# AssafSinger94/dino-tracker

Hardware: AMD Instinct MI355X
Metric: query-points*frames/s (higher is better)
Workload: dtype mixed: fp16 ViT operands (one per value), f16 conv operands in Delta-DINO, f16 candidates + f32 deciders in the tracker; f32 accumulate; 1 GPU; 854x480x90 synthetic video (model res 854x476, 67x121 tokens, C=384), 1024 grid queries; 1 video(s) per step over 1 GPU(s); features=vit, mode=single, track_method=mfma, anchor_pairs=92091, correlation_maps_per_video=8380350, rccl_ranks=1, parallelism=video-parallel x1

## Files before the change

### dino_tracker_amd/csrc/vit.hip

```cpp
#include <stdlib.h>
#include "common.h"
#include "vit_attention4.h"
#include "vit_attention6.h"
#include "vit_gemm_common.h"
#include "vit_gemm_tiled.h"
#include "vit_gemm_ws.h"
#include "vit_gemm_wide.h"
#include "vit_split.h"

namespace {

__global__ __launch_bounds__(256) void patch_embed_kernel(const float* __restrict__ frames, const float* __restrict__ Wp,
                                                          const float* __restrict__ bp, const float* __restrict__ pos,
                                                          const float* __restrict__ cls_pos,
                                                          const float* __restrict__ mean_std, float* __restrict__ x,
                                                          int H, int W, int ph, int pw, int D, int patch, int stride,
                                                          int S) {
    const int HW = ph * pw;
    const int K = 3 * patch * patch;
    const int frame = blockIdx.z;
    const int tid = threadIdx.x, lane = tid & 63, w = tid >> 6;
    const int p0 = blockIdx.x * 64 + (w >> 1) * 32;
    const int n0 = blockIdx.y * 64 + (w & 1) * 32;
    const int li = lane & 31, lk = lane >> 5;
    const float* img = frames + (size_t)frame * 3 * H * W;
    const int p = min(p0 + li, HW - 1);
    const int pr = p / pw, pc = p % pw;
    const int n = min(n0 + li, D - 1);
    const float* wrow = Wp + (size_t)n * K;
    f16v acc;
#pragma unroll
    for (int r = 0; r < 16; ++r) acc[r] = 0.f;
    for (int k = lk; k < K; k += 2) {
        const int ch = k / (patch * patch), rem = k - ch * patch * patch;
        const int ky = rem / patch, kx = rem - ky * patch;
        const float px = img[((size_t)ch * H + pr * stride + ky) * W + pc * stride + kx];
        const float a = (px - mean_std[ch]) / mean_std[3 + ch];
        acc = __builtin_amdgcn_mfma_f32_32x32x2f32(a, wrow[k], acc, 0, 0, 0);
    }
    const int co = n0 + li;
    if (co < D) {
        const float b = bp[co];
#pragma unroll
        for (int r = 0; r < 16; ++r) {
            const int i = (r & 3) + 8 * (r >> 2) + 4 * lk;
            const int pp = p0 + i;
            if (pp < HW) x[((size_t)frame * S + 1 + pp) * D + co] = acc[r] + b + pos[(size_t)pp * D + co];
        }
    }
    if (blockIdx.x == 0 && (w >> 1) == 0 && lk == 0 && co < D) x[(size_t)frame * S * D + co] = cls_pos[co];
}

constexpr int PE_P = 14, PE_S = 7, PE_TOK = 128, PE_NF = 96;
constexpr int PE_ROWPX = (PE_TOK - 1) * PE_S + PE_P;
constexpr int PE_K = PE_P * PE_P * 4;
constexpr int PE_CK = 2 * PE_P * 4;
constexpr int PE_WP = PE_CK + 8;
constexpr float PE_WSCALE = 256.f;

__global__ __launch_bounds__(256) void frame_split4_kernel(const float* __restrict__ frames, const float* __restrict__ mean_std,
                                                           h4v* __restrict__ hi_, h4v* __restrict__ lo_, int H, int W,
                                                           long long npix) {
    const long long i = (long long)blockIdx.x * 256 + threadIdx.x;
    if (i >= npix) return;
    const long long f = i / ((long long)H * W), p = i - f * (long long)H * W;
    const float* fr = frames + f * 3 * (long long)H * W + p;
    h4v h, l;
#pragma unroll
    for (int c = 0; c < 3; ++c) {
        const float v = (fr[(long long)c * H * W] - mean_std[c]) / mean_std[3 + c];
        h[c] = (half_t)v;
        l[c] = (half_t)(v - (float)h[c]);
    }
    h[3] = (half_t)0.f;
    l[3] = (half_t)0.f;
    hi_[i] = h;
    lo_[i] = l;
}

__global__ void pack_patch_split_kernel(const float* __restrict__ w, int D, half_t* __restrict__ Wh, half_t* __restrict__ Wl) {
    const long long idx = (long long)blockIdx.x * 256 + threadIdx.x;
    if (idx >= (long long)D * PE_K) return;
    const int n = (int)(idx / PE_K), k = (int)(idx - (long long)n * PE_K);
    const int tap = k >> 2, c = k & 3;
    const float v = c < 3 ? w[((size_t)n * 3 + c) * (PE_P * PE_P) + tap] * PE_WSCALE : 0.f;
    const half_t h = (half_t)v;
    Wh[idx] = h;
    Wl[idx] = (half_t)(v - (float)h);
}

__global__ __launch_bounds__(256) void patch_embed_split_kernel(const h4v* __restrict__ in_hi, const h4v* __restrict__ in_lo,
                                                                const half_t* __restrict__ Wh, const half_t* __restrict__ Wl,
                                                                const float* __restrict__ bp, const float* __restrict__ pos,
                                                                const float* __restrict__ cls_pos, float* __restrict__ x,
                                                                int H, int W, int ph, int pw, int D, int S, int groups_x,
                                                                int units, int slabs) {
    __shared__ h4v Xh[2 * PE_ROWPX], Xl[2 * PE_ROWPX];
    __shared__ __attribute__((aligned(16))) half_t Wsh[PE_NF * PE_WP], Wsl[PE_NF * PE_WP];
    const int tid = threadIdx.x, lane = tid & 63, w = tid >> 6;
    const int per_xcd = (units + 7) / 8;
    const int within = blockIdx.x >> 3;
    const int unit = (blockIdx.x & 7) * per_xcd + within / slabs;
    if (within / slabs >= per_xcd || unit >= units) return;
    const int n0 = (within % slabs) * PE_NF;
    const int pc0 = (unit % groups_x) * PE_TOK, pr = (unit / groups_x) % ph;
    const size_t frame = unit / (groups_x * ph);
    const int li = lane & 31, hh = lane >> 5;
    const h4v* fh = in_hi + frame * (size_t)H * W;
    const h4v* fl = in_lo + frame * (size_t)H * W;
    const int tokl = w * 32 + li;
    f16v acc[3];
#pragma unroll
    for (int n = 0; n < 3; ++n)
#pragma unroll
        for (int r = 0; r < 16; ++r) acc[n][r] = 0.f;
    for (int c = 0; c < PE_P / 2; ++c) {
        __syncthreads();
        for (int idx = tid; idx < 2 * PE_ROWPX; idx += 256) {
            const int r = idx / PE_ROWPX, px = idx - r * PE_ROWPX;
            const size_t g = (size_t)(pr * PE_S + 2 * c + r) * W + min(pc0 * PE_S + px, W - 1);
            Xh[idx] = fh[g];
            Xl[idx] = fl[g];
        }
        for (int idx = tid; idx < PE_NF * (PE_CK / 8); idx += 256) {
            const int f = idx / (PE_CK / 8), piece = idx - f * (PE_CK / 8);
            const size_t src = (size_t)min(n0 + f, D - 1) * PE_K + c * PE_CK + piece * 8;
            *reinterpret_cast<uint4*>(Wsh + f * PE_WP + piece * 8) = *reinterpret_cast<const uint4*>(Wh + src);
            *reinterpret_cast<uint4*>(Wsl + f * PE_WP + piece * 8) = *reinterpret_cast<const uint4*>(Wl + src);
        }
        __syncthreads();
#pragma unroll
        for (int ls = 0; ls < PE_CK / 16; ++ls) {
            const int t0 = 2 * (2 * ls + hh);
            const int p0 = (t0 / PE_P) * PE_ROWPX + tokl * PE_S + t0 % PE_P;
            const h4v a0 = Xh[p0], a1 = Xh[p0 + 1], b0 = Xl[p0], b1 = Xl[p0 + 1];
            const h8 xh = {a0[0], a0[1], a0[2], a0[3], a1[0], a1[1], a1[2], a1[3]};
            const h8 xl = {b0[0], b0[1], b0[2], b0[3], b1[0], b1[1], b1[2], b1[3]};
#pragma unroll
            for (int n = 0; n < 3; ++n) {
                const int wo = (n * 32 + li) * PE_WP + ls * 16 + hh * 8;
                const h8 wh = *reinterpret_cast<const h8*>(Wsh + wo), wl = *reinterpret_cast<const h8*>(Wsl + wo);
                acc[n] = __builtin_amdgcn_mfma_f32_32x32x16_f16(xl, wh, acc[n], 0, 0, 0);
                acc[n] = __builtin_amdgcn_mfma_f32_32x32x16_f16(xh, wl, acc[n], 0, 0, 0);
                acc[n] = __builtin_amdgcn_mfma_f32_32x32x16_f16(xh, wh, acc[n], 0, 0, 0);
            }
        }
    }
#pragma unroll
    for (int n = 0; n < 3; ++n) {
        const int co = n0 + n * 32 + li;
        if (co >= D) continue;
        const float b = bp[co];
#pragma unroll
        for (int r = 0; r < 16; ++r) {
            const int pc = pc0 + w * 32 + (r & 3) + 8 * (r >> 2) + 4 * hh;
            if (pc < pw) {
                const int pp = pr * pw + pc;
                x[((size_t)frame * S + 1 + pp) * D + co] = acc[n][r] * (1.f / PE_WSCALE) + b + pos[(size_t)pp * D + co];
            }
        }
        if (pr == 0 && pc0 == 0 && w == 0 && hh == 0) x[(size_t)frame * S * D + co] = cls_pos[co];
    }
}

template <typename T>
__global__ __launch_bounds__(256) void layernorm_kernel(float* __restrict__ x, const T* __restrict__ delta,
                                                        const float* __restrict__ gam, const float* __restrict__ bet,
                                                        T* __restrict__ y, long long rows, int D, float eps,
                                                        int* __restrict__ overflow) {
    typedef typename Vec<T>::t8 T8;
    typedef typename Vec<T>::t4 T4;
    (void)sizeof(T8); (void)sizeof(T4);
    operand_mode<T>();
    const long long row = (long long)blockIdx.x * 4 + (threadIdx.x >> 6);
    if (row >= rows) return;
    const int lane = threadIdx.x & 63;
    float* p = x + row * D;
    float4 v[4];
    float s = 0.f;
    bool sat = false;
#pragma unroll
    for (int it = 0; it < 4; ++it) {
        const int c = lane * 4 + it * 256;
        if (c < D) {
            v[it] = *reinterpret_cast<const float4*>(p + c);
            if (delta) {
                const T4 d = *reinterpret_cast<const T4*>(delta + row * D + c);
                const float d0 = (float)d[0], d1 = (float)d[1], d2 = (float)d[2], d3 = (float)d[3];
                if (IsF16<T>::value) sat |= !(fmaxf(fmaxf(fabsf(d0), fabsf(d1)), fmaxf(fabsf(d2), fabsf(d3))) < 65504.f);
                v[it].x += d0; v[it].y += d1; v[it].z += d2; v[it].w += d3;
                *reinterpret_cast<float4*>(p + c) = v[it];
            }
            s += (v[it].x + v[it].y) + (v[it].z + v[it].w);
        }
    }
    if (IsF16<T>::value && overflow && __any(sat) && lane == 0) atomicOr(overflow, 1);
    const float mean = wave_sum(s) / (float)D;
    float q = 0.f;
#pragma unroll
    for (int it = 0; it < 4; ++it) {
        if (lane * 4 + it * 256 < D) {
            const float a = v[it].x - mean, b = v[it].y - mean, cc = v[it].z - mean, d = v[it].w - mean;
            q += (a * a + b * b) + (cc * cc + d * d);
        }
    }
    const float rstd = rsqrtf(wave_sum(q) / (float)D + eps);
    if (!y) return;
    T* o = y + row * D;
#pragma unroll
    for (int it = 0; it < 4; ++it) {
        const int c = lane * 4 + it * 256;
        if (c < D) {
            const float4 g = *reinterpret_cast<const float4*>(gam + c), b = *reinterpret_cast<const float4*>(bet + c);
            T4 r = {(T)((v[it].x - mean) * rstd * g.x + b.x), (T)((v[it].y - mean) * rstd * g.y + b.y),
                     (T)((v[it].z - mean) * rstd * g.z + b.z), (T)((v[it].w - mean) * rstd * g.w + b.w)};
            *reinterpret_cast<T4*>(o + c) = r;
        }
    }
}

__global__ __launch_bounds__(256) void zero_kernel(uint4* __restrict__ p, long long n16) {
    const long long i = (long long)blockIdx.x * 256 + threadIdx.x;
    if (i < n16) p[i] = make_uint4(0, 0, 0, 0);
}

template <typename T>
__global__ __launch_bounds__(256) void final_update_kernel(const float* __restrict__ x, const T* __restrict__ delta,
                                                           float* __restrict__ tokens_out, float* __restrict__ feat_out, int S, int D,
                                                           long long total4, int* __restrict__ overflow) {
    typedef typename Vec<T>::t4 T4;
    const long long i = (long long)blockIdx.x * 256 + threadIdx.x;
    bool sat = false;
    if (i < total4) {
        const int d4 = D / 4;
        const long long row = i / d4;
        const int c = (int)(i - row * d4);
        const long long f = row / S, s = row - f * S;
        float4 v = reinterpret_cast<const float4*>(x)[i];
        const T4 d = reinterpret_cast<const T4*>(delta)[i];
        const float d0 = (float)d[0], d1 = (float)d[1], d2 = (float)d[2], d3 = (float)d[3];
        if (IsF16<T>::value) sat = !(fmaxf(fmaxf(fabsf(d0), fabsf(d1)), fmaxf(fabsf(d2), fabsf(d3))) < 65504.f);
        v.x += d0; v.y += d1; v.z += d2; v.w += d3;
        if (tokens_out) reinterpret_cast<float4*>(tokens_out)[i] = v;
        if (feat_out && s > 0) reinterpret_cast<float4*>(feat_out)[(f * (S - 1) + s - 1) * d4 + c] = v;
    }
    if (IsF16<T>::value && overflow && __any(sat) && (threadIdx.x & 63) == 0) atomicOr(overflow, 1);
}

template <typename T>
__global__ __launch_bounds__(256) void tap_kernel(const float* __restrict__ x, const T* __restrict__ delta, float* __restrict__ out,
                                                  float scale, long long total4) {
    typedef typename Vec<T>::t4 T4;
    const long long i = (long long)blockIdx.x * 256 + threadIdx.x;
    if (i >= total4) return;
    float4 v = reinterpret_cast<const float4*>(x)[i];
    if (delta) {
        const T4 d = reinterpret_cast<const T4*>(delta)[i];
        v.x += (float)d[0]; v.y += (float)d[1]; v.z += (float)d[2]; v.w += (float)d[3];
    }
    float4 o = reinterpret_cast<float4*>(out)[i];
    o.x += scale * v.x; o.y += scale * v.y; o.z += scale * v.z; o.w += scale * v.w;
    reinterpret_cast<float4*>(out)[i] = o;
}

__global__ __launch_bounds__(256) void drop_cls_kernel(const float* __restrict__ x, float* __restrict__ out, int S, int D,
                                                       long long total4) {
    const long long i = (long long)blockIdx.x * 256 + threadIdx.x;
    if (i >= total4) return;
    const int d4 = D / 4;
    const long long row = i / d4;
    const int c = (int)(i - row * d4);
    const long long f = row / (S - 1), s = row - f * (S - 1);
    reinterpret_cast<float4*>(out)[i] = reinterpret_cast<const float4*>(x)[(f * S + 1 + s) * d4 + c];
}

constexpr int VIT_FRAME_BATCH = 90;

struct VitPlan {
    int S, Sp, FB;
    size_t x, xn, q, k, vt, ao, hid, delta, total;
    bool split;
    size_t xn_lo, q_lo, k_lo, vt_lo, ao_lo, hid_lo;
};

inline bool vit_layer_split(const dtk_vit_layer& L) { return L.qkv_w_lo != nullptr; }

VitPlan vit_plan(const dtk_vit_model* m, int ph, int pw, int frames) {
    VitPlan p;
    p.S = ph * pw + 1;
    p.Sp = (p.S + 127) / 128 * 128;
    const int fb = m->frame_batch > 0 ? m->frame_batch : VIT_FRAME_BATCH;
    p.FB = frames < fb ? frames : fb;
    auto al = [](size_t v) { return (v + 255) & ~(size_t)255; };
    size_t off = 0;
    const size_t rows = (size_t)p.FB * p.S;
    p.x = off; off = al(off + rows * m->D * 4);
    p.xn = off; off = al(off + rows * m->D * 2);
    p.q = off; off = al(off + (size_t)p.FB * m->heads * p.Sp * 64 * 2);
    p.k = off; off = al(off + (size_t)p.FB * m->heads * p.Sp * 64 * 2);
    p.vt = off; off = al(off + (size_t)p.FB * m->heads * p.Sp * 64 * 2);
    p.ao = off; off = al(off + rows * m->D * 2);
    p.hid = off; off = al(off + rows * 4 * m->D * 2);
    p.delta = off; off = al(off + rows * m->D * 2);
    p.split = false;
    for (int l = 0; l < m->depth; ++l) p.split |= vit_layer_split(m->layers[l]);
    p.xn_lo = p.q_lo = p.k_lo = p.vt_lo = p.ao_lo = p.hid_lo = 0;
    if (p.split) {
        p.xn_lo = off; off = al(off + rows * m->D * 2);
        p.q_lo = off; off = al(off + (size_t)p.FB * m->heads * p.Sp * 64 * 2);
        p.k_lo = off; off = al(off + (size_t)p.FB * m->heads * p.Sp * 64 * 2);
        p.vt_lo = off; off = al(off + (size_t)p.FB * m->heads * p.Sp * 64 * 2);
        p.ao_lo = off; off = al(off + rows * m->D * 2);
        p.hid_lo = off; off = al(off + rows * 4 * m->D * 2);
    }
    p.total = off;
    return p;
}

template <typename T>
int attention_launch(const T* q, const T* k, const T* vt, T* o, int S, int Sp, int heads, int D, int FH, bool v4, hipStream_t st) {
    int QB;
    if (v4) {
        const unsigned grid = attn::attention_grid(FH, S, 256, &QB);
        DTK_LAUNCH("vit_attention", (attn::attention4_kernel<T, 0>), dim3(grid), dim3(256), 0, st, q, k, vt, o, S, Sp, heads, D,
                   FH, QB);
    } else {
        const unsigned grid = attn::attention_grid(FH, S, 128 * attn::A6_NQ, &QB);
        DTK_LAUNCH("vit_attention", (attn::attention6_kernel<T, 0>), dim3(grid), dim3(256), 0, st, q, k, vt, o, S, Sp, heads, D,
                   FH, QB);
    }
    return DTK_OK;
}

template <typename T>
__global__ __launch_bounds__(256) void range_scan_kernel(const T* __restrict__ p, long long n8, int* __restrict__ flag, int bit) {
    typedef typename Vec<T>::t8 T8;
    bool bad = false;
    for (long long i = (long long)blockIdx.x * 256 + threadIdx.x; i < n8; i += (long long)gridDim.x * 256) {
        const T8 v = reinterpret_cast<const T8*>(p)[i];
#pragma unroll
        for (int e = 0; e < 8; ++e) bad |= !(fabsf((float)v[e]) < 65504.f);
    }
    if (__any(bad) && (threadIdx.x & 63) == 0) atomicOr(flag, bit);
}

struct GemmPath {
    bool tiled;
    bool ws;
    bool wide;
    bool ws_v1;
    bool wide_v1;
    bool fc2_ln;
};
inline GemmPath gemm_path(int D, int f) {
    const bool tiled = (f & DTK_VIT_TILED_GEMMS) != 0, ws = !tiled && D == WS_K, wide_v1 = (f & DTK_VIT_GEMM_WIDE_V1) != 0;
    static_assert(WS_K == WD_N, "fc2 of the weight-stationary width is gemm_wide_delta_kernel's shape");
    return {tiled, ws, !tiled && D % W2_N == 0, (f & DTK_VIT_GEMM_WS_V1) != 0, wide_v1, ws && !wide_v1 && !(f & DTK_VIT_NO_LN_FUSION)};
}
inline GemmPath gemm_path(const dtk_vit_model* m) { return gemm_path(m->D, m->flags); }

template <typename T, int EPI>
int launch_gemm(const char* name, const GemmPath& path, const T* A, const T* W, long long rows, int N, int K, const GemmEpi<T>& e,
                hipStream_t st) {
    if constexpr (EPI != EPI_F32) {
        const bool ws_fits = EPI != EPI_QKV || e.S >= WS_ROWS || rows <= e.S;
        if (path.ws && K == WS_K && ws_fits) {
            const auto gr = gemm_ws_grid(N, rows);
            if (path.ws_v1)
                DTK_LAUNCH(name, (gemm_ws_kernel<T, EPI, 0>), gr.first, dim3(256), 0, st, A, W, rows, N, e, gr.second);
            else if (N % 64 != 0 || DTK_DBG(e.no_store, 128))
                DTK_LAUNCH(name, (gemm_ws_kernel<T, EPI, 3, false>), gr.first, dim3(256), 0, st, A, W, rows, N, e, gr.second);
            else
                DTK_LAUNCH(name, (gemm_ws_kernel<T, EPI>), gr.first, dim3(256), 0, st, A, W, rows, N, e, gr.second);
            return DTK_OK;
        }
        if (path.ws && EPI == EPI_DELTA) {
            const dim3 grid(dtk_cdiv(rows, WD_M));
            if (path.wide_v1)
                DTK_LAUNCH(name, (gemm_wide_delta_kernel<T, false>), grid, dim3(512), 0, st, A, W, rows, K, e);
            else if (e.ln_out)
                DTK_LAUNCH(name, (gemm_wide_delta_kernel<T, true, true>), grid, dim3(512), 0, st, A, W, rows, K, e);
            else
                DTK_LAUNCH(name, (gemm_wide_delta_kernel<T, true>), grid, dim3(512), 0, st, A, W, rows, K, e);
            return DTK_OK;
        }
        if (path.wide) {
            const dim3 grid(gemm_wide_grid(N, rows));
            if (path.wide_v1)
                DTK_LAUNCH(name, (gemm_wide_kernel<T, EPI, false>), grid, dim3(512), 0, st, A, W, rows, N, K, e);
            else
                DTK_LAUNCH(name, (gemm_wide_kernel<T, EPI, true>), grid, dim3(512), 0, st, A, W, rows, N, K, e);
            return DTK_OK;
        }
    }
    DTK_LAUNCH(name, (gemm_tiled_kernel<T, EPI>), dim3(gemm_grid(N, rows)), dim3(256), 0, st, A, W, rows, N, K, e);
    return DTK_OK;
}

template <typename T, int SEPI>
int launch_gemm_split(const char* name, const GemmPath& path, const T* Ah, const T* Al, const T* Wh, const T* Wl, long long rows,
                      int N, int K, const SplitEpi<T>& se, hipStream_t st) {
    if (!path.tiled && N % SD_N == 0) {
        const dim3 grid(gemm_split_dma_grid(N, rows));
        if (path.wide_v1)
            DTK_LAUNCH(name, (gemm_split_dma_kernel<T, SEPI, false>), grid, dim3(512), 0, st, Ah, Al, Wh, Wl, rows, N, K, se);
        else
            DTK_LAUNCH(name, (gemm_split_dma_kernel<T, SEPI, true>), grid, dim3(512), 0, st, Ah, Al, Wh, Wl, rows, N, K, se);
        return DTK_OK;
    }
    DTK_LAUNCH(name, (gemm_split_kernel<T, SEPI>), dim3(gemm_split_grid(N, rows)), dim3(256), 0, st, Ah, Al, Wh, Wl, rows, N, K, se);
    return DTK_OK;
}

template <typename T>
int vit_run(const dtk_vit_model* m, const float* frames, int nframes, int video_h, int video_w, float* tokens_out,
            float* feat_out, float* qkv_out, unsigned char* ws, const VitPlan& p, int ph, int pw, hipStream_t st) {
    const int HW = ph * pw, D = m->D;
    float* x = reinterpret_cast<float*>(ws + p.x);
    auto at = [&](size_t off) { return reinterpret_cast<T*>(ws + off); };
    T *xn = at(p.xn), *q = at(p.q), *k = at(p.k), *vt = at(p.vt), *ao = at(p.ao), *hid = at(p.hid), *delta = at(p.delta);
    T *xn_lo = at(p.xn_lo), *q_lo = at(p.q_lo), *k_lo = at(p.k_lo), *vt_lo = at(p.vt_lo), *ao_lo = at(p.ao_lo), *hid_lo = at(p.hid_lo);
    int* ovf = m->overflow;
    const bool scan_all = ovf && (m->flags & DTK_VIT_CHECK_RANGE);
    int* const epi_ovf = IsF16<T>::value ? ovf : nullptr;
    const int S = p.S, Sp = p.Sp;
    {
        const long long n16 = (long long)((p.ao - p.q) / 16);
        DTK_LAUNCH("vit_zero", zero_kernel, dim3(dtk_cdiv(n16, 256)), dim3(256), 0, st, reinterpret_cast<uint4*>(q), n16);
        if (p.split) {
            const long long m16 = (long long)((p.ao_lo - p.q_lo) / 16);
            DTK_LAUNCH("vit_zero", zero_kernel, dim3(dtk_cdiv(m16, 256)), dim3(256), 0, st, reinterpret_cast<uint4*>(q_lo), m16);
        }
    }
    for (int f0 = 0; f0 < nframes; f0 += p.FB) {
        const int nf = (nframes - f0) < p.FB ? (nframes - f0) : p.FB;
        const long long rows = (long long)nf * S;
        auto scan_range = [&](const T* t, long long n, int bit) -> int {
            const int blocks = (int)(dtk_cdiv(n / 8, 256) < 1024 ? dtk_cdiv(n / 8, 256) : 1024);
            DTK_LAUNCH("vit_range_scan", range_scan_kernel<T>, dim3(blocks), dim3(256), 0, st, t, n / 8, ovf, bit);
            return DTK_OK;
        };
        const bool pe_fits = (size_t)nf * video_h * video_w * 16 <= p.delta - p.hid &&
                             (size_t)D * PE_K * 4 <= p.total - p.delta;
        if (m->patch == PE_P && m->stride == PE_S && pe_fits) {
            h4v* fh = reinterpret_cast<h4v*>(hid);
            h4v* fl = fh + (size_t)nf * video_h * video_w;
            half_t* wh = reinterpret_cast<half_t*>(delta);
            half_t* wl = wh + (size_t)D * PE_K;
            const long long npix = (long long)nf * video_h * video_w;
            DTK_LAUNCH("vit_frame_split", frame_split4_kernel, dim3(dtk_cdiv(npix, 256)), dim3(256), 0, st,
                       frames + (size_t)f0 * 3 * video_h * video_w, m->mean_std, fh, fl, video_h, video_w, npix);
            DTK_LAUNCH("vit_frame_split", pack_patch_split_kernel, dim3(dtk_cdiv((long long)D * PE_K, 256)), dim3(256), 0, st,
                       m->patch_w, D, wh, wl);
            const int groups_x = dtk_cdiv(pw, PE_TOK);
            const int units = groups_x * ph * nf, slabs = dtk_cdiv(D, PE_NF);
            DTK_LAUNCH("vit_patch_embed", patch_embed_split_kernel, dim3(8 * dtk_cdiv(units, 8) * slabs), dim3(256), 0, st, fh,
                       fl, wh, wl, m->patch_b, m->pos, m->cls_pos, x, video_h, video_w, ph, pw, D, S, groups_x, units, slabs);
        } else {
            DTK_LAUNCH("vit_patch_embed", patch_embed_kernel, dim3(dtk_cdiv(HW, 64), dtk_cdiv(D, 64), nf), dim3(256), 0, st,
                       frames + (size_t)f0 * 3 * video_h * video_w, m->patch_w, m->patch_b, m->pos, m->cls_pos, m->mean_std,
                       x, video_h, video_w, ph, pw, D, m->patch, m->stride, S);
        }
        const GemmPath path = gemm_path(m);
        const int dbg_ns = DTK_DBG(dtk_dev_flags() >> 16, 0xff);
        bool pending = false;
        bool ln1_done = false;
        auto tap = [&](int l, bool with_delta) -> int {
            if (!m->tap_out || !((m->tap_mask >> l) & 1)) return DTK_OK;
            const long long t4 = rows * (D / 4);
            DTK_LAUNCH("vit_tap", tap_kernel<T>, dim3(dtk_cdiv(t4, 256)), dim3(256), 0, st, x, with_delta ? (const T*)delta : (const T*)nullptr,
                       m->tap_out + (size_t)f0 * S * D, m->tap_scale, t4);
            return DTK_OK;
        };
        for (int l = 0; l < m->depth; ++l) {
            const dtk_vit_layer& L = m->layers[l];
            const T* qkv_w = reinterpret_cast<const T*>(L.qkv_w);
            const T* proj_w = reinterpret_cast<const T*>(L.proj_w);
            const T* fc1_w = reinterpret_cast<const T*>(L.fc1_w);
            const T* fc2_w = reinterpret_cast<const T*>(L.fc2_w);
            if (vit_layer_split(L)) {
                const T* qkv_wl = reinterpret_cast<const T*>(L.qkv_w_lo);
                const T* proj_wl = reinterpret_cast<const T*>(L.proj_w_lo);
                const T* fc1_wl = reinterpret_cast<const T*>(L.fc1_w_lo);
                const T* fc2_wl = reinterpret_cast<const T*>(L.fc2_w_lo);
                const float inv_ws = 1.f / (L.w_scale > 0.f ? L.w_scale : 1.f);
                DTK_LAUNCH("vit_layernorm_split", layernorm_split_kernel<T>, dim3(dtk_cdiv(rows, 4)), dim3(256), 0, st, x,
                           pending ? (const T*)delta : (const T*)nullptr, L.ln1_w, L.ln1_b, xn, xn_lo, rows, D, m->ln_eps, ovf);
                pending = false;
                SplitEpi<T> se{};
                if (qkv_out && l == m->depth - 1) {
                    se.bias = L.qkv_b; se.inv_wscale = inv_ws; se.out_f32 = qkv_out + (size_t)f0 * S * 3 * D;
                    if (launch_gemm_split<T, SEPI_F32>("vit_gemm_qkv_facet", path, xn, xn_lo, qkv_w, qkv_wl, rows, 3 * D, D, se, st)) return DTK_E_HIP;
                    se = SplitEpi<T>{};
                }
                se.bias = L.qkv_b; se.inv_wscale = inv_ws; se.q_hi = q; se.q_lo = q_lo; se.k_hi = k; se.k_lo = k_lo; se.vt_hi = vt;
                se.vt_lo = vt_lo; se.S = S; se.Sp = Sp; se.heads = m->heads; se.D = D; se.qscale = 0.125f * 1.4426950408889634f;
                se.ovf = epi_ovf;
                if (launch_gemm_split<T, SEPI_QKV>("vit_gemm_qkv_split", path, xn, xn_lo, qkv_w, qkv_wl, rows, 3 * D, D, se, st)) return DTK_E_HIP;
                const int nqb = dtk_cdiv(Sp, 128);
                DTK_LAUNCH("vit_attention_split", attention_split_kernel<T>, dim3((unsigned)(nf * m->heads * nqb)), dim3(256), 0, st,
                           (const T*)q, (const T*)q_lo, (const T*)k, (const T*)k_lo, (const T*)vt, (const T*)vt_lo, ao, ao_lo, S, Sp,
                           m->heads, nqb);
                se = SplitEpi<T>{};
                se.bias = L.proj_b; se.inv_wscale = inv_ws; se.x = x; se.gamma = L.ls1;
                if (launch_gemm_split<T, SEPI_RESID>("vit_gemm_proj_split", path, ao, ao_lo, proj_w, proj_wl, rows, D, D, se, st)) return DTK_E_HIP;
                DTK_LAUNCH("vit_layernorm_split", layernorm_split_kernel<T>, dim3(dtk_cdiv(rows, 4)), dim3(256), 0, st, x,
                           (const T*)nullptr, L.ln2_w, L.ln2_b, xn, xn_lo, rows, D, m->ln_eps, ovf);
                se = SplitEpi<T>{};
                se.bias = L.fc1_b; se.inv_wscale = inv_ws; se.out_hi = hid; se.out_lo = hid_lo; se.ovf = epi_ovf;
                if (launch_gemm_split<T, SEPI_GELU>("vit_gemm_fc1_split", path, xn, xn_lo, fc1_w, fc1_wl, rows, 4 * D, D, se, st)) return DTK_E_HIP;
                se = SplitEpi<T>{};
                se.bias = L.fc2_b; se.inv_wscale = inv_ws; se.x = x; se.gamma = L.ls2;
                if (launch_gemm_split<T, SEPI_RESID>("vit_gemm_fc2_split", path, hid, hid_lo, fc2_w, fc2_wl, rows, D, 4 * D, se, st)) return DTK_E_HIP;
                if (tap(l, false)) return DTK_E_HIP;
                continue;
            }
            GemmEpi<T> e{};
            if (!ln1_done)
                DTK_LAUNCH("vit_layernorm", layernorm_kernel<T>, dim3(dtk_cdiv(rows, 4)), dim3(256), 0, st, x,
                           pending ? (const T*)delta : (const T*)nullptr, L.ln1_w, L.ln1_b, xn, rows, D, m->ln_eps, ovf);
            ln1_done = false;
            pending = true;
            if (qkv_out && l == m->depth - 1) {
                e.bias = L.qkv_b; e.out_f32 = qkv_out + (size_t)f0 * S * 3 * D;
                if (launch_gemm<T, EPI_F32>("vit_gemm_qkv_facet", path, xn, qkv_w, rows, 3 * D, D, e, st)) return DTK_E_HIP;
                e = GemmEpi<T>{};
            }
            e.bias = L.qkv_b; e.q = q; e.k = k; e.vt = vt; e.S = S; e.Sp = Sp; e.heads = m->heads; e.D = D;
            e.qscale = 0.125f * 1.4426950408889634f; e.no_store = dbg_ns; e.ovf = epi_ovf;
            if (launch_gemm<T, EPI_QKV>("vit_gemm_qkv", path, xn, qkv_w, rows, 3 * D, D, e, st)) return DTK_E_HIP;
            if (scan_all && scan_range(q, (long long)(p.ao - p.q) / 2, 2)) return DTK_E_HIP;
            if (attention_launch(q, k, vt, ao, S, Sp, m->heads, D, nf * m->heads, (m->flags & DTK_VIT_ATTENTION_V4) != 0, st)) return DTK_E_HIP;
            e = GemmEpi<T>{};
            e.bias = L.proj_b; e.delta = delta; e.gamma = L.ls1; e.no_store = dbg_ns;
            if (launch_gemm<T, EPI_DELTA>("vit_gemm_proj", path, ao, proj_w, rows, D, D, e, st)) return DTK_E_HIP;
            DTK_LAUNCH("vit_layernorm", layernorm_kernel<T>, dim3(dtk_cdiv(rows, 4)), dim3(256), 0, st, x, (const T*)delta,
                       L.ln2_w, L.ln2_b, xn, rows, D, m->ln_eps, ovf);
            e = GemmEpi<T>{};
            e.bias = L.fc1_b; e.out = hid; e.no_store = dbg_ns; e.ovf = epi_ovf;
            if (launch_gemm<T, EPI_GELU>("vit_gemm_fc1", path, xn, fc1_w, rows, 4 * D, D, e, st)) return DTK_E_HIP;
            if (scan_all && scan_range(hid, rows * 4 * D, 4)) return DTK_E_HIP;
            e = GemmEpi<T>{};
            e.bias = L.fc2_b; e.delta = delta; e.gamma = L.ls2; e.no_store = dbg_ns;
            if (path.fc2_ln && l + 1 < m->depth && !vit_layer_split(m->layers[l + 1])) {
                const dtk_vit_layer& Ln = m->layers[l + 1];
                e.ln_x = x; e.ln_w = Ln.ln1_w; e.ln_b = Ln.ln1_b; e.ln_out = xn; e.ln_eps = m->ln_eps; e.ln_ovf = ovf;
                pending = false;
                ln1_done = true;
            }
            if (launch_gemm<T, EPI_DELTA>("vit_gemm_fc2", path, hid, fc2_w, rows, D, 4 * D, e, st)) return DTK_E_HIP;
            if (tap(l, pending)) return DTK_E_HIP;
        }
        if (pending && (tokens_out || feat_out)) {
            const long long t4 = rows * (D / 4);
            DTK_LAUNCH("vit_final_update", final_update_kernel<T>, dim3(dtk_cdiv(t4, 256)), dim3(256), 0, st, x, (const T*)delta,
                       tokens_out ? tokens_out + (size_t)f0 * S * D : (float*)nullptr,
                       feat_out ? feat_out + (size_t)f0 * HW * D : (float*)nullptr, S, D, t4, ovf);
        } else {
            if (pending)
                DTK_LAUNCH("vit_layernorm", layernorm_kernel<T>, dim3(dtk_cdiv(rows, 4)), dim3(256), 0, st, x, (const T*)delta,
                           (const float*)nullptr, (const float*)nullptr, (T*)nullptr, rows, D, m->ln_eps, ovf);
            if (tokens_out)
                DTK_HIP(hipMemcpyAsync(tokens_out + (size_t)f0 * S * D, x, (size_t)rows * D * sizeof(float),
                                       hipMemcpyDeviceToDevice, st));
            if (feat_out) {
                const long long total4 = (long long)nf * HW * (D / 4);
                DTK_LAUNCH("vit_drop_cls", drop_cls_kernel, dim3(dtk_cdiv(total4, 256)), dim3(256), 0, st, x,
                           feat_out + (size_t)f0 * HW * D, S, D, total4);
            }
        }
    }
    return DTK_OK;
}

int vit_gemm_check(const dtk_vit_gemm_args* g, const char* who, bool split, int* N, int* K) {
    DTK_REQUIRE(g, "%s: null pointer", who);
    DTK_REQUIRE(g->D == 384 || g->D == 768 || g->D == 1024, "%s: D must be 384, 768 or 1024 (got %d)", who, g->D);
    DTK_REQUIRE(g->operand_type == DTK_OPERAND_F16 || g->operand_type == DTK_OPERAND_BF16, "%s: operand_type", who);
    DTK_REQUIRE(g->rows > 0 && g->rows < (1ll << 31), "%s: rows", who);
    DTK_REQUIRE(g->a && g->w && (!split || (g->a_lo && g->w_lo)), "%s: null operand", who);
    const int D = g->D;
    switch (g->role) {
        case DTK_VIT_GEMM_QKV:
            *N = 3 * D; *K = D;
            DTK_REQUIRE(g->q && g->k && g->vt && (!split || (g->q_lo && g->k_lo && g->vt_lo)), "%s: QKV needs q, k and vt", who);
            DTK_REQUIRE(g->S > 0 && g->Sp >= g->S && g->Sp % 64 == 0 && g->rows % g->S == 0,
                        "%s: bad sizes (Sp %% 64 == 0, Sp >= S, rows a multiple of S)", who);
            break;
        case DTK_VIT_GEMM_QKV_FACET:
            *N = 3 * D; *K = D;
            DTK_REQUIRE(g->out_f32, "%s: QKV_FACET needs out_f32", who);
            break;
        case DTK_VIT_GEMM_FC1:
            *N = 4 * D; *K = D;
            DTK_REQUIRE(g->out && (!split || g->out_lo), "%s: FC1 needs out", who);
            break;
        case DTK_VIT_GEMM_PROJ:
        case DTK_VIT_GEMM_FC2:
            *N = D; *K = g->role == DTK_VIT_GEMM_FC2 ? 4 * D : D;
            DTK_REQUIRE(g->gamma && (split ? g->x != nullptr : g->out != nullptr), "%s: PROJ / FC2 need gamma and %s", who, split ? "x" : "out");
            break;
        default:
            DTK_REQUIRE(false, "%s: unknown role %d", who, g->role);
    }
    return DTK_OK;
}

template <typename T>
int vit_gemm_stage(const dtk_vit_gemm_args* g, int N, int K, hipStream_t st) {
    const GemmPath path = gemm_path(g->D, g->flags);
    const T *A = reinterpret_cast<const T*>(g->a), *W = reinterpret_cast<const T*>(g->w);
    int* const epi_ovf = IsF16<T>::value ? g->ovf : nullptr;
    GemmEpi<T> e{};
    e.bias = g->bias;
    switch (g->role) {
        case DTK_VIT_GEMM_QKV:
            e.q = reinterpret_cast<T*>(g->q); e.k = reinterpret_cast<T*>(g->k); e.vt = reinterpret_cast<T*>(g->vt);
            e.S = g->S; e.Sp = g->Sp; e.heads = g->D / 64; e.D = g->D; e.qscale = 0.125f * 1.4426950408889634f; e.ovf = epi_ovf;
            return launch_gemm<T, EPI_QKV>("vit_gemm_qkv", path, A, W, g->rows, N, K, e, st);
        case DTK_VIT_GEMM_QKV_FACET:
            e.out_f32 = g->out_f32;
            return launch_gemm<T, EPI_F32>("vit_gemm_qkv_facet", path, A, W, g->rows, N, K, e, st);
        case DTK_VIT_GEMM_FC1:
            e.out = reinterpret_cast<T*>(g->out); e.ovf = epi_ovf;
            return launch_gemm<T, EPI_GELU>("vit_gemm_fc1", path, A, W, g->rows, N, K, e, st);
        default:
            e.delta = reinterpret_cast<T*>(g->out); e.gamma = g->gamma;
            if (g->ln_out) {
                DTK_REQUIRE(g->role == DTK_VIT_GEMM_FC2 && path.fc2_ln, "dtk_vit_gemm: the fused LayerNorm is fc2's at D = 384 without TILED_GEMMS / GEMM_WIDE_V1 / NO_LN_FUSION");
                DTK_REQUIRE(g->ln_x && g->ln_w && g->ln_b, "dtk_vit_gemm: the fused LayerNorm needs ln_x, ln_w and ln_b");
                e.ln_x = g->ln_x; e.ln_w = g->ln_w; e.ln_b = g->ln_b; e.ln_out = reinterpret_cast<T*>(g->ln_out); e.ln_eps = g->ln_eps;
                e.ln_ovf = g->ovf;
            }
            return launch_gemm<T, EPI_DELTA>(g->role == DTK_VIT_GEMM_PROJ ? "vit_gemm_proj" : "vit_gemm_fc2", path, A, W, g->rows, N, K, e, st);
    }
}

template <typename T>
int vit_gemm_split_stage(const dtk_vit_gemm_args* g, int N, int K, hipStream_t st) {
    const GemmPath path = gemm_path(g->D, g->flags);
    const T *Ah = reinterpret_cast<const T*>(g->a), *Al = reinterpret_cast<const T*>(g->a_lo);
    const T *Wh = reinterpret_cast<const T*>(g->w), *Wl = reinterpret_cast<const T*>(g->w_lo);
    int* const epi_ovf = IsF16<T>::value ? g->ovf : nullptr;
    SplitEpi<T> se{};
    se.bias = g->bias; se.inv_wscale = 1.f / (g->w_scale > 0.f ? g->w_scale : 1.f);
    switch (g->role) {
        case DTK_VIT_GEMM_QKV:
            se.q_hi = reinterpret_cast<T*>(g->q); se.q_lo = reinterpret_cast<T*>(g->q_lo); se.k_hi = reinterpret_cast<T*>(g->k);
            se.k_lo = reinterpret_cast<T*>(g->k_lo); se.vt_hi = reinterpret_cast<T*>(g->vt); se.vt_lo = reinterpret_cast<T*>(g->vt_lo);
            se.S = g->S; se.Sp = g->Sp; se.heads = g->D / 64; se.D = g->D; se.qscale = 0.125f * 1.4426950408889634f; se.ovf = epi_ovf;
            return launch_gemm_split<T, SEPI_QKV>("vit_gemm_qkv_split", path, Ah, Al, Wh, Wl, g->rows, N, K, se, st);
        case DTK_VIT_GEMM_QKV_FACET:
            se.out_f32 = g->out_f32;
            return launch_gemm_split<T, SEPI_F32>("vit_gemm_qkv_facet", path, Ah, Al, Wh, Wl, g->rows, N, K, se, st);
        case DTK_VIT_GEMM_FC1:
            se.out_hi = reinterpret_cast<T*>(g->out); se.out_lo = reinterpret_cast<T*>(g->out_lo); se.ovf = epi_ovf;
            return launch_gemm_split<T, SEPI_GELU>("vit_gemm_fc1_split", path, Ah, Al, Wh, Wl, g->rows, N, K, se, st);
        default:
            se.x = g->x; se.gamma = g->gamma;
            return launch_gemm_split<T, SEPI_RESID>(g->role == DTK_VIT_GEMM_PROJ ? "vit_gemm_proj_split" : "vit_gemm_fc2_split", path, Ah, Al,
                                                    Wh, Wl, g->rows, N, K, se, st);
    }
}

constexpr int VIT_KNOWN_FLAGS = DTK_VIT_TILED_GEMMS | DTK_VIT_BF16 | DTK_VIT_CHECK_RANGE | DTK_VIT_GEMM_WS_V1 | DTK_VIT_ATTENTION_V4 |
                                DTK_VIT_GEMM_WIDE_V1 | DTK_VIT_NO_LN_FUSION;

}

extern "C" size_t dtk_vit_workspace_bytes(const dtk_vit_model* m, int video_h, int video_w, int frames) {
    if (!m || frames <= 0) return 0;
    const int ph = 1 + (video_h - m->patch) / m->stride, pw = 1 + (video_w - m->patch) / m->stride;
    return vit_plan(m, ph, pw, frames).total;
}

extern "C" int dtk_vit_forward(const dtk_vit_model* m, const float* frames, int nframes, int video_h, int video_w,
                               float* tokens_out, float* feat_out, float* qkv_out, void* workspace,
                               size_t workspace_bytes, void* stream) {
    DTK_REQUIRE(m && frames && workspace && (tokens_out || feat_out || qkv_out || m->tap_out), "dtk_vit_forward: null pointer");
    DTK_REQUIRE(!(m->flags & ~VIT_KNOWN_FLAGS), "dtk_vit_forward: unknown flag bits 0x%x (bit 8 selected a kernel that left the library)",
                (unsigned)(m->flags & ~VIT_KNOWN_FLAGS));
    DTK_REQUIRE(!qkv_out || m->depth > 0, "dtk_vit_forward: qkv_out needs at least one block");
    DTK_REQUIRE(m->D > 0 && m->heads > 0 && m->D == m->heads * 64, "dtk_vit_forward: d_head must be 64 (D=%d heads=%d)",
                m->D, m->heads);
    DTK_REQUIRE(m->D % 32 == 0 && m->depth >= 0 && m->layers, "dtk_vit_forward: bad model");
    DTK_REQUIRE(video_h >= m->patch && video_w >= m->patch, "dtk_vit_forward: frame smaller than a patch");
    const int ph = 1 + (video_h - m->patch) / m->stride, pw = 1 + (video_w - m->patch) / m->stride;
    const VitPlan p = vit_plan(m, ph, pw, nframes);
    if (workspace_bytes < p.total) {
        dtk_set_error("dtk_vit_forward: workspace %zu B < required %zu B", workspace_bytes, p.total);
        return DTK_E_WORKSPACE;
    }
    hipStream_t st = dtk_stream(stream);
    unsigned char* ws = reinterpret_cast<unsigned char*>(workspace);
    if (m->flags & DTK_VIT_BF16)
        return vit_run<__bf16>(m, frames, nframes, video_h, video_w, tokens_out, feat_out, qkv_out, ws, p, ph, pw, st);
    return vit_run<_Float16>(m, frames, nframes, video_h, video_w, tokens_out, feat_out, qkv_out, ws, p, ph, pw, st);
}

extern "C" int dtk_vit_attention(const void* q, const void* k, const void* vt, void* out, int frames, int heads, int S,
                                 int Sp, int operand_type, void* stream) {
    DTK_REQUIRE(q && k && vt && out, "dtk_vit_attention: null pointer");
    DTK_REQUIRE(frames > 0 && heads > 0 && S > 0 && Sp >= S && Sp % 64 == 0, "dtk_vit_attention: bad sizes (Sp %% 64 == 0, Sp >= S)");
    const bool v4 = (operand_type & DTK_OPERAND_ATTENTION_V4) != 0;
    operand_type &= ~DTK_OPERAND_ATTENTION_V4;
    DTK_REQUIRE(operand_type == DTK_OPERAND_F16 || operand_type == DTK_OPERAND_BF16, "dtk_vit_attention: operand_type");
    if (operand_type == DTK_OPERAND_BF16)
        return attention_launch(reinterpret_cast<const __bf16*>(q), reinterpret_cast<const __bf16*>(k),
                                reinterpret_cast<const __bf16*>(vt), reinterpret_cast<__bf16*>(out), S, Sp, heads, heads * 64,
                                frames * heads, v4, dtk_stream(stream));
    return attention_launch(reinterpret_cast<const _Float16*>(q), reinterpret_cast<const _Float16*>(k),
                            reinterpret_cast<const _Float16*>(vt), reinterpret_cast<_Float16*>(out), S, Sp, heads, heads * 64,
                            frames * heads, v4, dtk_stream(stream));
}

extern "C" int dtk_vit_attention_split(const void* q_hi, const void* q_lo, const void* k_hi, const void* k_lo, const void* vt_hi,
                                       const void* vt_lo, void* out_hi, void* out_lo, int frames, int heads, int S, int Sp,
                                       int operand_type, void* stream) {
    DTK_REQUIRE(q_hi && q_lo && k_hi && k_lo && vt_hi && vt_lo && out_hi && out_lo, "dtk_vit_attention_split: null pointer");
    DTK_REQUIRE(frames > 0 && heads > 0 && S > 0 && Sp >= S && Sp % 64 == 0, "dtk_vit_attention_split: bad sizes (Sp %% 64 == 0, Sp >= S)");
    DTK_REQUIRE(operand_type == DTK_OPERAND_F16 || operand_type == DTK_OPERAND_BF16, "dtk_vit_attention_split: operand_type");
    hipStream_t st = dtk_stream(stream);
    const int nqb = dtk_cdiv(Sp, 128);
    const unsigned grid = (unsigned)(frames * heads * nqb);
    if (operand_type == DTK_OPERAND_BF16) {
        typedef __bf16 T;
        DTK_LAUNCH("vit_attention_split", attention_split_kernel<T>, dim3(grid), dim3(256), 0, st, (const T*)q_hi, (const T*)q_lo,
                   (const T*)k_hi, (const T*)k_lo, (const T*)vt_hi, (const T*)vt_lo, (T*)out_hi, (T*)out_lo, S, Sp, heads, nqb);
    } else {
        typedef _Float16 T;
        DTK_LAUNCH("vit_attention_split", attention_split_kernel<T>, dim3(grid), dim3(256), 0, st, (const T*)q_hi, (const T*)q_lo,
                   (const T*)k_hi, (const T*)k_lo, (const T*)vt_hi, (const T*)vt_lo, (T*)out_hi, (T*)out_lo, S, Sp, heads, nqb);
    }
    return DTK_OK;
}


extern "C" int dtk_vit_gemm(const dtk_vit_gemm_args* g, void* stream) {
    int N = 0, K = 0;
    if (const int rc = vit_gemm_check(g, "dtk_vit_gemm", false, &N, &K)) return rc;
    if (g->operand_type == DTK_OPERAND_BF16) return vit_gemm_stage<__bf16>(g, N, K, dtk_stream(stream));
    return vit_gemm_stage<_Float16>(g, N, K, dtk_stream(stream));
}

extern "C" int dtk_vit_gemm_split(const dtk_vit_gemm_args* g, void* stream) {
    int N = 0, K = 0;
    if (const int rc = vit_gemm_check(g, "dtk_vit_gemm_split", true, &N, &K)) return rc;
    DTK_REQUIRE(!g->ln_out, "dtk_vit_gemm_split: the split blocks have their own LayerNorm");
    if (g->operand_type == DTK_OPERAND_BF16) return vit_gemm_split_stage<__bf16>(g, N, K, dtk_stream(stream));
    return vit_gemm_split_stage<_Float16>(g, N, K, dtk_stream(stream));
}
```

Before: 529,400 query-points*frames/s.

## Fuse residual update and LayerNorm2 into the weight-stationary projection GEMM

Measured after the change: 534,700 query-points*frames/s, median of 6. +1.0%, better.

```diff
diff --git a/dino_tracker_amd/csrc/vit.hip b/dino_tracker_amd/csrc/vit.hip
--- a/dino_tracker_amd/csrc/vit.hip
+++ b/dino_tracker_amd/csrc/vit.hip
@@ -5,6 +5,7 @@
 #include "vit_gemm_common.h"
 #include "vit_gemm_tiled.h"
 #include "vit_gemm_ws.h"
+#include "vit_gemm_ws_ln.h"
 #include "vit_gemm_wide.h"
 #include "vit_split.h"
 
@@ -351,11 +352,13 @@
     bool ws_v1;
     bool wide_v1;
     bool fc2_ln;
+    bool proj_ln;
 };
 inline GemmPath gemm_path(int D, int f) {
     const bool tiled = (f & DTK_VIT_TILED_GEMMS) != 0, ws = !tiled && D == WS_K, wide_v1 = (f & DTK_VIT_GEMM_WIDE_V1) != 0;
     static_assert(WS_K == WD_N, "fc2 of the weight-stationary width is gemm_wide_delta_kernel's shape");
-    return {tiled, ws, !tiled && D % W2_N == 0, (f & DTK_VIT_GEMM_WS_V1) != 0, wide_v1, ws && !wide_v1 && !(f & DTK_VIT_NO_LN_FUSION)};
+    const bool ws_v1 = (f & DTK_VIT_GEMM_WS_V1) != 0, fc2_ln = ws && !wide_v1 && !(f & DTK_VIT_NO_LN_FUSION);
+    return {tiled, ws, !tiled && D % W2_N == 0, ws_v1, wide_v1, fc2_ln, fc2_ln && !ws_v1};
 }
 inline GemmPath gemm_path(const dtk_vit_model* m) { return gemm_path(m->D, m->flags); }
 
@@ -364,6 +367,13 @@
                 hipStream_t st) {
     if constexpr (EPI != EPI_F32) {
         const bool ws_fits = EPI != EPI_QKV || e.S >= WS_ROWS || rows <= e.S;
+        if constexpr (EPI == EPI_DELTA) {
+            if (path.ws && K == WS_K && N == WS_K && e.ln_out) {
+                const auto gr = gemm_ws_ln_grid(rows);
+                DTK_LAUNCH(name, (gemm_ws_ln_kernel<T>), gr.first, dim3(256), 0, st, A, W, rows, e, gr.second);
+                return DTK_OK;
+            }
+        }
         if (path.ws && K == WS_K && ws_fits) {
             const auto gr = gemm_ws_grid(N, rows);
             if (path.ws_v1)
@@ -533,9 +543,11 @@
             if (attention_launch(q, k, vt, ao, S, Sp, m->heads, D, nf * m->heads, (m->flags & DTK_VIT_ATTENTION_V4) != 0, st)) return DTK_E_HIP;
             e = GemmEpi<T>{};
             e.bias = L.proj_b; e.delta = delta; e.gamma = L.ls1; e.no_store = dbg_ns;
+            if (path.proj_ln) { e.ln_x = x; e.ln_w = L.ln2_w; e.ln_b = L.ln2_b; e.ln_out = xn; e.ln_eps = m->ln_eps; e.ln_ovf = ovf; }
             if (launch_gemm<T, EPI_DELTA>("vit_gemm_proj", path, ao, proj_w, rows, D, D, e, st)) return DTK_E_HIP;
-            DTK_LAUNCH("vit_layernorm", layernorm_kernel<T>, dim3(dtk_cdiv(rows, 4)), dim3(256), 0, st, x, (const T*)delta,
-                       L.ln2_w, L.ln2_b, xn, rows, D, m->ln_eps, ovf);
+            if (!path.proj_ln)
+                DTK_LAUNCH("vit_layernorm", layernorm_kernel<T>, dim3(dtk_cdiv(rows, 4)), dim3(256), 0, st, x, (const T*)delta,
+                           L.ln2_w, L.ln2_b, xn, rows, D, m->ln_eps, ovf);
             e = GemmEpi<T>{};
             e.bias = L.fc1_b; e.out = hid; e.no_store = dbg_ns; e.ovf = epi_ovf;
             if (launch_gemm<T, EPI_GELU>("vit_gemm_fc1", path, xn, fc1_w, rows, 4 * D, D, e, st)) return DTK_E_HIP;
@@ -627,7 +639,8 @@
         default:
             e.delta = reinterpret_cast<T*>(g->out); e.gamma = g->gamma;
             if (g->ln_out) {
-                DTK_REQUIRE(g->role == DTK_VIT_GEMM_FC2 && path.fc2_ln, "dtk_vit_gemm: the fused LayerNorm is fc2's at D = 384 without TILED_GEMMS / GEMM_WIDE_V1 / NO_LN_FUSION");
+                DTK_REQUIRE(g->role == DTK_VIT_GEMM_FC2 ? path.fc2_ln : path.proj_ln,
+                            "dtk_vit_gemm: the fused LayerNorm is fc2's or the projection's at D = 384 without TILED_GEMMS / GEMM_WIDE_V1 / NO_LN_FUSION (the projection's: nor GEMM_WS_V1)");
                 DTK_REQUIRE(g->ln_x && g->ln_w && g->ln_b, "dtk_vit_gemm: the fused LayerNorm needs ln_x, ln_w and ln_b");
                 e.ln_x = g->ln_x; e.ln_w = g->ln_w; e.ln_b = g->ln_b; e.ln_out = reinterpret_cast<T*>(g->ln_out); e.ln_eps = g->ln_eps;
                 e.ln_ovf = g->ovf;
diff --git a/dino_tracker_amd/csrc/vit_gemm_ws_ln.h b/dino_tracker_amd/csrc/vit_gemm_ws_ln.h
--- /dev/null
+++ b/dino_tracker_amd/csrc/vit_gemm_ws_ln.h
@@ -0,0 +1,199 @@
+#pragma once
+#include <utility>
+#include "vit_gemm_ws.h"
+
+namespace {
+
+constexpr int WL_N = WS_K;
+constexpr int WL_WCOLS = WL_N / 4;
+constexpr int WL_RT = WL_WCOLS / 32;
+constexpr int WL_AGPR_FRAGS = 60;
+constexpr int WL_PITCH = WL_N * 2 + 16;
+constexpr int WL_STAGE_BYTES = WS_ROWS * WL_PITCH;
+constexpr int WL_MAX_TPC = 65536;
+static_assert(WL_RT * 32 * 4 == WL_N, "four waves of whole 32-row weight tiles");
+
+template <typename T>
+__global__ __launch_bounds__(256) void gemm_ws_ln_kernel(const T* __restrict__ A, const T* __restrict__ Wt, long long M, GemmEpi<T> e,
+                                                         int tiles_per_chunk) {
+    typedef typename Vec<T>::t8 T8;
+    typedef typename Vec<T>::t4 T4;
+    (void)sizeof(T8); (void)sizeof(T4);
+    operand_mode<T>();
+    __shared__ __attribute__((aligned(1024))) unsigned char toks[3][WS_TILE_BYTES];
+    __shared__ __attribute__((aligned(16))) unsigned char stage[2][WL_STAGE_BYTES];
+    __shared__ __attribute__((aligned(16))) float s_bias[WL_N], s_gamma[WL_N];
+    const int tid = threadIdx.x, lane = tid & 63;
+    const int w = __builtin_amdgcn_readfirstlane(tid >> 6);
+    const int j = lane & 31, h = lane >> 5;
+    const int n0 = w * WL_WCOLS;
+    const long long total_tiles = (M + WS_ROWS - 1) / WS_ROWS;
+    const long long tile0 = (long long)blockIdx.x * tiles_per_chunk;
+    if (tile0 >= total_tiles) return;
+    const int NT = (int)((total_tiles - tile0) < tiles_per_chunk ? (total_tiles - tile0) : tiles_per_chunk);
+    const int nl = (j & 3) + 4 * (j >> 3) + 16 * ((j >> 2) & 1);
+    T8 wf[WL_RT][WS_KS];
+#pragma unroll
+    for (int t = 0; t < WL_RT; ++t) {
+        const T* wp = Wt + (size_t)(n0 + t * 32 + nl) * WS_K + h * 8;
+#pragma unroll
+        for (int ks = 0; ks < WS_KS; ++ks) {
+            if (t * WS_KS + ks < WL_AGPR_FRAGS) asm volatile("global_load_dwordx4 %0, %1, off" : "=a"(wf[t][ks]) : "v"(wp + ks * 16) : "memory");
+            else wf[t][ks] = *reinterpret_cast<const T8*>(wp + ks * 16);
+        }
+    }
+    asm volatile("s_waitcnt vmcnt(0)" ::: "memory");
+#pragma unroll
+    for (int t = 0; t < WL_RT; ++t)
+#pragma unroll
+        for (int ks = 0; ks < WS_KS; ++ks)
+            if (t * WS_KS + ks < WL_AGPR_FRAGS) asm volatile("" : "+a"(wf[t][ks]));
+    for (int i = tid; i < WL_N; i += 256) {
+        s_bias[i] = e.bias ? e.bias[i] : 0.f;
+        s_gamma[i] = e.gamma[i];
+    }
+    const f4 ga = *reinterpret_cast<const f4*>(e.ln_w + lane * 4), ba = *reinterpret_cast<const f4*>(e.ln_b + lane * 4);
+    const f4 gb = *reinterpret_cast<const f4*>(e.ln_w + 256 + (lane & 31) * 4), bb = *reinterpret_cast<const f4*>(e.ln_b + 256 + (lane & 31) * 4);
+    asm volatile("" ::"v"(ga), "v"(ba), "v"(gb), "v"(bb));
+    const unsigned lds_base = (unsigned)(size_t)&toks[0][0];
+    const int l_tt = lane & 3, l_pp = lane >> 2;
+    const dtk_u4 srd = dtk_make_srd(A + tile0 * WS_ROWS * WS_K);
+    unsigned a_voff[2], a_voff_last[2];
+    const int last_rows = (int)(M - (total_tiles - 1) * WS_ROWS);
+#pragma unroll
+    for (int gg = 0; gg < 2; ++gg) {
+        const int g = 2 * w + gg;
+        a_voff[gg] = (unsigned)(((4 * g + l_tt) * WS_K + ((l_pp - g) & 15) * 8) * 2);
+        a_voff_last[gg] = (unsigned)((min(4 * g + l_tt, last_rows - 1) * WS_K + ((l_pp - g) & 15) * 8) * 2);
+    }
+    const unsigned a_dst = __builtin_amdgcn_readfirstlane(lds_base + (2 * w) * 3 * 1024);
+    auto issue = [&](int n, int buf) {
+        const unsigned toff = __builtin_amdgcn_readfirstlane((unsigned)n * (unsigned)WS_TILE_BYTES);
+        const unsigned dst = __builtin_amdgcn_readfirstlane(a_dst + (unsigned)buf * (unsigned)WS_TILE_BYTES);
+        const bool last = tile0 + n == total_tiles - 1;
+        const unsigned v0 = last ? a_voff_last[0] : a_voff[0], v1 = last ? a_voff_last[1] : a_voff[1];
+        dtk_buffer_lds16<0>(srd, toff, v0, dst);
+        dtk_buffer_lds16<1024>(srd, toff + 256u, v0, dst);
+        dtk_buffer_lds16<2048>(srd, toff + 512u, v0, dst);
+        dtk_buffer_lds16<3072>(srd, toff, v1, dst);
+        dtk_buffer_lds16<4096>(srd, toff + 256u, v1, dst);
+        dtk_buffer_lds16<5120>(srd, toff + 512u, v1, dst);
+    };
+    unsigned frag_off[8];
+#pragma unroll
+    for (int k8 = 0; k8 < 8; ++k8)
+        frag_off[k8] = (unsigned)((j >> 2) * 3 * 1024 + ((((2 * k8 + h + (j >> 2)) & 15) * 4 + (j & 3)) * 16));
+    bool sat = false;
+    issue(0, 0);
+    issue(min(1, NT - 1), 1);
+    dtk_vm_wait<WS_LQ>();
+    __syncthreads();
+    int b0 = 0;
+    for (int n = 0; n < NT; ++n) {
+        const int b2 = b0 == 0 ? 2 : b0 - 1;
+        const long long rb = (tile0 + n) * WS_ROWS + 8 * w;
+        f4 xa[8], xb[8];
+#pragma unroll
+        for (int rr = 0; rr < 8; ++rr) {
+            const float* xp = e.ln_x + min(rb + rr, M - 1) * WL_N;
+            asm volatile("global_load_dwordx4 %0, %1, off" : "=v"(xa[rr]) : "v"(xp + lane * 4) : "memory");
+            asm volatile("global_load_dwordx4 %0, %1, off" : "=v"(xb[rr]) : "v"(xp + 256 + (lane & 31) * 4) : "memory");
+        }
+        issue(min(n + 2, NT - 1), b2);
+        f16v acc[WL_RT];
+        {
+            const unsigned char* base = &toks[0][0] + b0 * WS_TILE_BYTES;
+            const f16v zero16 = {0.f, 0.f, 0.f, 0.f, 0.f, 0.f, 0.f, 0.f, 0.f, 0.f, 0.f, 0.f, 0.f, 0.f, 0.f, 0.f};
+            T8 b[3];
+            b[0] = *reinterpret_cast<const T8*>(base + frag_off[0]);
+            b[1] = *reinterpret_cast<const T8*>(base + frag_off[1]);
+#pragma unroll
+            for (int ks = 0; ks < WS_KS; ++ks) {
+                if (ks + 2 < WS_KS)
+                    b[(ks + 2) % 3] = *reinterpret_cast<const T8*>(base + frag_off[(ks + 2) & 7] + ((ks + 2) >> 3) * 1024);
+#pragma unroll
+                for (int t = 0; t < WL_RT; ++t) acc[t] = mfma32(wf[t][ks], b[ks % 3], ks == 0 ? zero16 : acc[t]);
+            }
+        }
+        {
+            unsigned char* const sw = &stage[n & 1][0] + j * WL_PITCH + (n0 + 16 * h) * 2;
+#pragma unroll
+            for (int t = 0; t < WL_RT; ++t)
+#pragma unroll
+                for (int hv = 0; hv < 2; ++hv) {
+                    const int fb = n0 + 32 * t + 16 * h + 8 * hv;
+                    const float4 b0v = *reinterpret_cast<const float4*>(&s_bias[fb]), b1v = *reinterpret_cast<const float4*>(&s_bias[fb + 4]);
+                    const float4 g0v = *reinterpret_cast<const float4*>(&s_gamma[fb]), g1v = *reinterpret_cast<const float4*>(&s_gamma[fb + 4]);
+                    const float bi[8] = {b0v.x, b0v.y, b0v.z, b0v.w, b1v.x, b1v.y, b1v.z, b1v.w};
+                    const float gm[8] = {g0v.x, g0v.y, g0v.z, g0v.w, g1v.x, g1v.y, g1v.z, g1v.w};
+                    T8 o;
+#pragma unroll
+                    for (int r = 0; r < 8; ++r) {
+                        const float v0 = acc[t][8 * hv + r] + bi[r];
+                        o[r] = (T)(v0 * gm[r]);
+                    }
+                    *reinterpret_cast<T8*>(sw + 64 * t + 16 * hv) = o;
+                }
+        }
+        dtk_vm_wait<WS_LQ>();
+#pragma unroll
+        for (int rr = 0; rr < 8; ++rr) asm volatile("" : "+v"(xa[rr]), "+v"(xb[rr]));
+        __syncthreads();
+#pragma unroll
+        for (int rr = 0; rr < 8; ++rr) {
+            const long long row = rb + rr;
+            if (row >= M) continue;
+            const unsigned char* sp = &stage[n & 1][0] + (8 * w + rr) * WL_PITCH + lane * 8;
+            f4 v[2] = {xa[rr], xb[rr]};
+            float s = 0.f;
+#pragma unroll
+            for (int it = 0; it < 2; ++it) {
+                if (it == 0 || lane < 32) {
+                    const T4 d = *reinterpret_cast<const T4*>(sp + it * 512);
+                    const float d0 = (float)d[0], d1 = (float)d[1], d2 = (float)d[2], d3 = (float)d[3];
+                    if (IsF16<T>::value) sat |= !(fmaxf(fmaxf(fabsf(d0), fabsf(d1)), fmaxf(fabsf(d2), fabsf(d3))) < 65504.f);
+                    v[it].x += d0; v[it].y += d1; v[it].z += d2; v[it].w += d3;
+                    *reinterpret_cast<f4*>(e.ln_x + row * WL_N + it * 256 + lane * 4) = v[it];
+                    s += (v[it].x + v[it].y) + (v[it].z + v[it].w);
+                }
+            }
+            const float mean = wave_sum(s) / (float)WL_N;
+            float q = 0.f;
+#pragma unroll
+            for (int it = 0; it < 2; ++it) {
+                if (it == 0 || lane < 32) {
+                    const float a = v[it].x - mean, b = v[it].y - mean, cc = v[it].z - mean, d = v[it].w - mean;
+                    q += (a * a + b * b) + (cc * cc + d * d);
+                }
+            }
+            const float rstd = rsqrtf(wave_sum(q) / (float)WL_N + e.ln_eps);
+            T* o = e.ln_out + row * WL_N;
+#pragma unroll
+            for (int it = 0; it < 2; ++it) {
+                if (it == 0 || lane < 32) {
+                    const f4 g = it ? gb : ga, b = it ? bb : ba;
+                    T4 r = {(T)((v[it].x - mean) * rstd * g.x + b.x), (T)((v[it].y - mean) * rstd * g.y + b.y),
+                             (T)((v[it].z - mean) * rstd * g.z + b.z), (T)((v[it].w - mean) * rstd * g.w + b.w)};
+                    *reinterpret_cast<T4*>(o + it * 256 + lane * 4) = r;
+                }
+            }
+        }
+        b0 = b0 == 2 ? 0 : b0 + 1;
+    }
+    if (IsF16<T>::value && e.ln_ovf && __any(sat) && lane == 0) atomicOr(e.ln_ovf, 1);
+    dtk_vm_wait<0>();
+}
+
+inline std::pair<dim3, int> gemm_ws_ln_grid(long long rows) {
+    static const int cus = [] {
+        int dev = 0, n = 0;
+        if (hipGetDevice(&dev) != hipSuccess || hipDeviceGetAttribute(&n, hipDeviceAttributeMultiprocessorCount, dev) != hipSuccess || n <= 0) n = 256;
+        return n;
+    }();
+    const long long tiles = dtk_cdiv(rows, WS_ROWS);
+    int tpc = (int)dtk_cdiv(tiles, cus);
+    if (tpc > WL_MAX_TPC) tpc = WL_MAX_TPC;
+    return std::make_pair(dim3((unsigned)dtk_cdiv(tiles, tpc)), tpc);
+}
+
+}
```
